# wenz116/lang2seg

Measured on AMD Instinct MI355X. Metric: train images/sec (cycle loss on), 600×1000 input, at 1/2/4/8 MI355X, higher is better.
Workload: dtype bf16; 1 GPU; train_cycle.sh step: ResNet-101 C4 + 7 spatial dynamic filters + att2in2 cycle loss, 600x1000 image, 20-token expression (V=3349), 12000->2000 proposals, 256 RoIs, per-GPU batch 1; variant=cycle, parallelism=dp1

## Files before the change

lang2seg_amd/csrc/conv_igemm.hip:

```cpp
#include "common.h"
#include "roi_sample.h"
#include "../../include/lang2seg_hip.h"
#include <stdlib.h>

namespace {

template <typename T> struct Mma;
template <> struct Mma<bf16_t> {
  static __device__ __forceinline__ f32x4 run(const uint4& a, const uint4& b, f32x4 c) {
    return __builtin_amdgcn_mfma_f32_16x16x32_bf16(__builtin_bit_cast(bf16x8, a), __builtin_bit_cast(bf16x8, b), c, 0, 0, 0);
  }
};
template <> struct Mma<float> {
  static __device__ __forceinline__ f32x4 run(const uint4& a, const uint4& b, f32x4 c) {
    c = __builtin_amdgcn_mfma_f32_16x16x4f32(__uint_as_float(a.x), __uint_as_float(b.x), c, 0, 0, 0);
    c = __builtin_amdgcn_mfma_f32_16x16x4f32(__uint_as_float(a.y), __uint_as_float(b.y), c, 0, 0, 0);
    c = __builtin_amdgcn_mfma_f32_16x16x4f32(__uint_as_float(a.z), __uint_as_float(b.z), c, 0, 0, 0);
    c = __builtin_amdgcn_mfma_f32_16x16x4f32(__uint_as_float(a.w), __uint_as_float(b.w), c, 0, 0, 0);
    return c;
  }
};

constexpr int ROWB = 128;
constexpr int LROW = ROWB + 16;
// ... 699 lines not shown
    __syncthreads();
    int t0 = 0;
    for (; t0 + 2 * D <= KT; t0 += D) {
#pragma unroll
      for (int s = 0; s < D; ++s) {
        const int t = t0 + s;
        const int nxt = (s + 1) % D;
        store_slice((t + 1) & 1, ra[nxt], rb[nxt]);
        issue(ra[nxt], rb[nxt]);
        __syncthreads();
      }
    }
#pragma unroll
    for (int s = 0; s < 2 * D; ++s) {
      const int t = t0 + s;
      if (t + 1 < KT) {
        const int nxt = (s + 1) % D;
        store_slice((t + 1) & 1, ra[nxt], rb[nxt]);
        if (t + 1 + D < KT) issue(ra[nxt], rb[nxt]);
        __syncthreads();
      }
    }
    return;
  }

  const int tid = (int)threadIdx.x, lane = tid & 63, wave = wave_all;
  const int wm = wave >> 1, wn = wave & 1;
  const int fr = lane & 15, fg = lane >> 4;
  const bool plain = !(p.flags & (L2S_CONV_DECONV2X2 | L2S_CONV_SCATTER)) && !(p.ldy & 7) && !(p.ldadd & 7) && !(p.ldref & 7) && !(p.Cout & 7) &&
                     !((uintptr_t)p.y & 15) && !((uintptr_t)p.add & 15) && !((uintptr_t)p.ref & 15) && !((uintptr_t)p.bias & 15) &&
                     (long)M * p.ldy * 2 < (1L << 31) && (!p.add || (long)M * p.ldadd * 2 < (1L << 31)) && (!p.ref || (long)M * p.ldref * 2 < (1L << 31));
  const bool staged = plain && gridDim.z == 1;
  constexpr int EIT = (BM * (BN / 8) + 255) / 256;
  u32x4v eav[EIT], erv[EIT];
  const bool pre = staged;
  if (pre && KT >= 8) igemm_epilogue_prefetch<BM, 256, BN>(p, m0, n0, M, tid, eav, erv);
  f32x4 ebv[BN / 32];
#pragma unroll
  for (int j = 0; j < BN / 32; ++j) {
    const int n = n0 + (wave_all & 1) * (BN / 2) + j * 16 + (lane >> 4) * 4;
    ebv[j] = (f32x4){0.f, 0.f, 0.f, 0.f};
    if (staged && p.bias && n < p.Cout) ebv[j] = *(const f32x4*)(p.bias + n);
  }
  const int swz = fr & (CPR - 1);
  const int offa = (wm * WM + fr) * RB, offb = BM * RB + (wn * WN + fr) * RB;
  f32x4 acc[TM][TN];
#pragma unroll
  for (int i = 0; i < TM; ++i)
#pragma unroll
    for (int j = 0; j < TN; ++j) acc[i][j] = (f32x4){0.f, 0.f, 0.f, 0.f};
  uint4 fa0[KG][TM], fb0[KG][TN], fa1[KG][TM], fb1[KG][TN];
  auto read_all = [&](int t, uint4 (&fa)[KG][TM], uint4 (&fb)[KG][TN]) {
    const char* base = smem + (t & 1) * BUF;
#pragma unroll
    for (int kg = 0; kg < KG; ++kg) {
      const int ch = ((kg * 4 + fg) ^ swz) << 4;
#pragma unroll
      for (int i = 0; i < TM; ++i) fa[kg][i] = *(const uint4*)(base + offa + i * 16 * RB + ch);
#pragma unroll
      for (int j = 0; j < TN; ++j) fb[kg][j] = *(const uint4*)(base + offb + j * 16 * RB + ch);
    }
  };
  auto mma_all = [&](const uint4 (&fa)[KG][TM], const uint4 (&fb)[KG][TN]) {
#pragma unroll
    for (int kg = 0; kg < KG; ++kg)
#pragma unroll
      for (int i = 0; i < TM; ++i)
#pragma unroll
        for (int j = 0; j < TN; ++j) acc[i][j] = Mma<T>::run(fb[kg][j], fa[kg][i], acc[i][j]);
  };
  __syncthreads();
  unsigned long long t_first = 0, t_loop = 0;
  if constexpr (STAMP) t_first = __builtin_amdgcn_s_memrealtime();
  read_all(0, fa0, fb0);
  if (pre && KT < 8) igemm_epilogue_prefetch<BM, 256, BN>(p, m0, n0, M, tid, eav, erv);
  int t = 1;
  for (; t + 2 <= KT; t += 2) {
    __syncthreads(); read_all(t, fa1, fb1); mma_all(fa0, fb0);
    __syncthreads(); read_all(t + 1, fa0, fb0); mma_all(fa1, fb1);
  }
  if (t < KT) { __syncthreads(); read_all(t, fa1, fb1); mma_all(fa0, fb0); mma_all(fa1, fb1); }
  else mma_all(fa0, fb0);
  if (gridDim.z > 1) { igemm_splitk_slab<TM, TN, WM, WN>(p, acc, m0, n0, wm, wn, fr, fg, M); return; }
  if constexpr (STAMP) {
    asm volatile("s_nop 0" : "+v"(acc[0][0]), "+v"(acc[TM - 1][TN - 1]));
    t_loop = __builtin_amdgcn_s_memrealtime();
  }
  if (staged) {
    igemm_epilogue_lds128<TM, TN, WM, WN, 2, 256, BN, 1>(p, acc, m0, n0, wm, wn, fr, fg, M, smem_all, eav, erv, ebv);
    if constexpr (STAMP) {
      asm volatile("s_waitcnt vmcnt(0)" ::: "memory");
      if (tid == 0 && p.ws) {
        unsigned long long* o = (unsigned long long*)p.ws + 4L * (blockIdx.x + (long)gridDim.x * blockIdx.z);
        o[0] = t_entry; o[1] = t_first; o[2] = t_loop; o[3] = __builtin_amdgcn_s_memrealtime();
      }
    }
    return;
  }
  igemm_epilogue<T, TM, TN, WM, WN, false>(p, acc, m0, n0, wm, wn, fr, fg, M);
}

template <typename T, int BM, int BN, int WGM, int WGN, int D, bool OUTF32, bool TAPIN>
__global__ __launch_bounds__(64 * WGM * WGN) void igemm_sp_kernel(const l2s_conv_desc p) {
  constexpr int VE = 16 / (int)sizeof(T);
  constexpr int BK = ROWB / (int)sizeof(T);
  constexpr int NTG = 64 * WGM * WGN, LR = NTG / 8;
  constexpr int WM = BM / WGM, WN = BN / WGN, TM = WM / 16, TN = WN / 16;
  constexpr int NA = (BM + LR - 1) / LR, NB = BN / LR;
  constexpr int BUF = (BM + BN) * ROWB;
  static_assert(D >= 2, "ring depth");
  extern __shared__ __attribute__((aligned(16))) char smem[];

  const int tid = threadIdx.x, lane = tid & 63, wave = tid >> 6;
  const int wm = wave / WGN, wn = wave % WGN;
  const int M = p.n_img * p.OH * p.OW;
  const int K = p.KH * p.KW * p.Cin;
  int mt, nt;
  {
    const int MT = (M + BM - 1) / BM, NT = (p.Cout + BN - 1) / BN, G = MT * NT;
    const int L = blockIdx.x, x = L & 7, slot = L >> 3, q = G >> 3, r = G & 7;
    const int t = x * q + min(x, r) + slot;
    if (p.xcd_mode == 0) { mt = t / NT; nt = t - mt * NT; } else { nt = t / MT; mt = t - nt * MT; }
  }
  const int m0 = mt * BM, n0 = nt * BN;
  const long xpix = (long)p.n_img * p.IH * p.IW;
  const auto rx = __builtin_amdgcn_make_buffer_rsrc((void*)p.x, 0, (int)(((xpix - 1) * p.ldx + p.Cin) * (long)sizeof(T)), 0x00020000);
  const auto rw = __builtin_amdgcn_make_buffer_rsrc((void*)p.w, 0, (int)((long)p.Cout * K * (long)sizeof(T)), 0x00020000);

  const int lrow = tid >> 3, cv = tid & 7;
  const int wchunk = ((cv ^ (lrow & 7)) << 4);
  int a_iy0[NA], a_ix0[NA], a_base[NA]; bool a_ok[NA];
  const int ohw = p.OH * p.OW;
#pragma unroll
  for (int j = 0; j < NA; ++j) {
    int m = m0 + lrow + LR * j;
    a_ok[j] = m < M && (lrow + LR * j) < BM;
    int mm = a_ok[j] ? m : 0;
    int n_img = mm / ohw, rem = mm - n_img * ohw;
    int oy = rem / p.OW, ox = rem - oy * p.OW;
    a_iy0[j] = oy * p.stride - p.pad;
    a_ix0[j] = ox * p.stride - p.pad;
    a_base[j] = n_img * p.IH * p.IW;
  }
  unsigned voffB[NB];
#pragma unroll
  for (int j = 0; j < NB; ++j) {
    const int n = n0 + lrow + LR * j;
    voffB[j] = n < p.Cout ? (unsigned)(((long)n * K + cv * VE) * (long)sizeof(T)) : OOR;
  }
  const int KT = K / BK;
  const int taps = p.KH * p.KW;
  int it = 0, c0 = 0, tap = 0;
  unsigned voffA[NA];
  int vbase[NA]; unsigned tmask[NA];
  auto set_tap = [&](int t) {
    const int ky = t / p.KW, kx = t - ky * p.KW;
#pragma unroll
    for (int j = 0; j < NA; ++j) {
      const int iy = a_iy0[j] + ky, ix = a_ix0[j] + kx;
      const bool v = a_ok[j] && iy >= 0 && iy < p.IH && ix >= 0 && ix < p.IW;
      voffA[j] = v ? (unsigned)(((long)(a_base[j] + iy * p.IW + ix) * p.ldx + cv * VE) * (long)sizeof(T)) : OOR;
    }
  };
  if (TAPIN) {
#pragma unroll
    for (int j = 0; j < NA; ++j) {
      vbase[j] = ((a_base[j] + a_iy0[j] * p.IW + a_ix0[j]) * p.ldx + cv * VE) * (int)sizeof(T);
      unsigned m = 0;
      for (int t = 0; t < taps; ++t) {
        const int ky = t / p.KW, kx = t - ky * p.KW;
        const int iy = a_iy0[j] + ky, ix = a_ix0[j] + kx;
        if (a_ok[j] && iy >= 0 && iy < p.IH && ix >= 0 && ix < p.IW) m |= 1u << t;
      }
      tmask[j] = m;
    }
  } else {
    set_tap(0);
  }
  auto issue = [&](uint4 (&a)[NA], uint4 (&b)[NB]) {
    int sa, sb;
    if (TAPIN) {
      const int ky = tap / p.KW, kx = tap - ky * p.KW;
      const int toff = (ky * p.IW + kx) * p.ldx * (int)sizeof(T);
      sa = c0 * (int)sizeof(T); sb = (tap * p.Cin + c0) * (int)sizeof(T);
#pragma unroll
      for (int j = 0; j < NA; ++j) voffA[j] = ((tmask[j] >> tap) & 1u) ? (unsigned)(vbase[j] + toff) : OOR;
    } else {
      sa = c0 * (int)sizeof(T); sb = it * (BK * (int)sizeof(T));
    }
#pragma unroll
    for (int j = 0; j < NA; ++j) a[j] = __builtin_bit_cast(uint4, __builtin_amdgcn_raw_buffer_load_b128(rx, voffA[j], sa, 0));
#pragma unroll
    for (int j = 0; j < NB; ++j) b[j] = __builtin_bit_cast(uint4, __builtin_amdgcn_raw_buffer_load_b128(rw, voffB[j], sb, 0));
    ++it;
    if (TAPIN) {
      if (++tap == taps) { tap = 0; c0 += BK; }
    } else {
      c0 += BK;
      if (c0 >= p.Cin && taps > 1) { c0 = 0; ++tap; if (tap < taps) set_tap(tap); }
    }
  };
  auto store_slice = [&](int buf, const uint4 (&ra)[NA], const uint4 (&rb)[NB]) {
    char* a = smem + buf * BUF + lrow * ROWB + wchunk;
    char* b = a + BM * ROWB;
#pragma unroll
    for (int j = 0; j < NA; ++j) if ((BM % LR) == 0 || j < NA - 1 || lrow < (BM % LR)) *(uint4*)(a + LR * j * ROWB) = ra[j];
#pragma unroll
    for (int j = 0; j < NB; ++j) *(uint4*)(b + LR * j * ROWB) = rb[j];
  };

  f32x4 acc[TM][TN];
#pragma unroll
  for (int i = 0; i < TM; ++i)
#pragma unroll
    for (int j = 0; j < TN; ++j) acc[i][j] = (f32x4){0.f, 0.f, 0.f, 0.f};

  const int fr = lane & 15, fg = lane >> 4;
  const int swz = fr & 7;
  const int offa = (wm * WM + fr) * ROWB, offb = BM * ROWB + (wn * WN + fr) * ROWB;
  const int ch0 = ((0 * 4 + fg) ^ swz) << 4, ch1 = ((1 * 4 + fg) ^ swz) << 4;
  auto read_frags = [&](int buf, int ch, uint4 (&fa)[TM], uint4 (&fb)[TN]) {
    const char* base = smem + buf * BUF;
#pragma unroll
    for (int i = 0; i < TM; ++i) fa[i] = *(const uint4*)(base + offa + i * 16 * ROWB + ch);
#pragma unroll
    for (int j = 0; j < TN; ++j) fb[j] = *(const uint4*)(base + offb + j * 16 * ROWB + ch);
  };
  auto mma = [&](const uint4 (&fa)[TM], const uint4 (&fb)[TN]) {
#pragma unroll
    for (int i = 0; i < TM; ++i)
#pragma unroll
      for (int j = 0; j < TN; ++j) acc[i][j] = Mma<T>::run(fb[j], fa[i], acc[i][j]);
  };

  uint4 ra[D][NA], rb[D][NB];
#pragma unroll
  for (int s = 0; s < D; ++s)
    if (s < KT) issue(ra[s], rb[s]);
  store_slice(0, ra[0], rb[0]);
  if (D < KT) issue(ra[0], rb[0]);
  if (1 < KT) {
    store_slice(1, ra[1], rb[1]);
    if (D + 1 < KT) issue(ra[1], rb[1]);
  }
  __syncthreads();
  uint4 fa0[TM], fb0[TN], fa1[TM], fb1[TN];
  read_frags(0, ch0, fa0, fb0);

  int t0 = 0, b0 = 0;
  for (; t0 + 2 * D + 2 <= KT; t0 += D) {
#pragma unroll
    for (int s = 0; s < D; ++s) {
      const int set = (s + 2) % D;
      const int bt = b0, bt1 = b0 == 2 ? 0 : b0 + 1, bt2 = bt1 == 2 ? 0 : bt1 + 1;
      if (s > 0 || t0 > 0) __syncthreads();
      read_frags(bt, ch1, fa1, fb1);
      store_slice(bt2, ra[set], rb[set]);
      issue(ra[set], rb[set]);
      mma(fa0, fb0);
      read_frags(bt1, ch0, fa0, fb0);
      mma(fa1, fb1);
      b0 = bt1;
    }
  }
#pragma unroll
  for (int s = 0; s < 2 * D + 2; ++s) {
    const int t = t0 + s;
    if (t < KT) {
      const int set = (s + 2) % D;
      const int bt = b0, bt1 = b0 == 2 ? 0 : b0 + 1, bt2 = bt1 == 2 ? 0 : bt1 + 1;
      if (t > 0) __syncthreads();
      read_frags(bt, ch1, fa1, fb1);
      if (t + 2 < KT) {
        store_slice(bt2, ra[set], rb[set]);
        if (t + 2 + D < KT) issue(ra[set], rb[set]);
      }
      mma(fa0, fb0);
      if (t + 1 < KT) read_frags(bt1, ch0, fa0, fb0);
      mma(fa1, fb1);
      b0 = bt1;
    }
  }
  if constexpr (sizeof(T) == 2 && !OUTF32 && BN == 128) {
    const bool plain = !(p.flags & (L2S_CONV_DECONV2X2 | L2S_CONV_SCATTER)) && !(p.ldy & 7) && !(p.ldadd & 7) && !(p.ldref & 7) && !(p.Cout & 7) &&
                       !((uintptr_t)p.y & 15) && !((uintptr_t)p.add & 15) && !((uintptr_t)p.ref & 15) && !((uintptr_t)p.bias & 15) &&
                       (long)M * p.ldy * 2 < (1L << 31) && (!p.add || (long)M * p.ldadd * 2 < (1L << 31)) && (!p.ref || (long)M * p.ldref * 2 < (1L << 31));
    if (plain) { igemm_epilogue_lds128<TM, TN, WM, WN, WGM, NTG, BN, 1>(p, acc, m0, n0, wm, wn, fr, fg, M, smem); return; }
  }
  igemm_epilogue<T, TM, TN, WM, WN, OUTF32>(p, acc, m0, n0, wm, wn, fr, fg, M);
}

typedef int i32x4s __attribute__((ext_vector_type(4)));
__device__ __forceinline__ void dma_b128(const i32x4s& rsrc, unsigned voff, unsigned soff, unsigned lds) {
  asm volatile("s_mov_b32 m0, %3\n\ts_nop 0\n\tbuffer_load_dwordx4 %0, %1, %2 offen lds" ::"v"(voff), "s"(rsrc), "s"(soff), "s"(lds) : "memory");
}
__device__ __forceinline__ void wg_barrier() { asm volatile("s_barrier" ::: "memory"); }
__device__ __forceinline__ void wait_lgkm0() { asm volatile("s_waitcnt lgkmcnt(0)" ::: "memory"); }

template <int BM, int BN, bool STAMP = false>
__global__ __launch_bounds__(512) void igemm_dma_kernel(const l2s_conv_desc p) {
  typedef bf16_t T;
  constexpr int WGM = 4, WGN = 2, WM = BM / WGM, WN = BN / WGN, TM = WM / 16, TN = WN / 16;
  constexpr int PA = BM / 64, PB = BN / 64, NP = PA + PB;
  constexpr int STG = (BM + BN) * ROWB;
  extern __shared__ __attribute__((aligned(16))) char smem[];
  const int tid = threadIdx.x, lane = tid & 63;
  const int wave = __builtin_amdgcn_readfirstlane(tid >> 6);
  const int grp = wave >> 2;
  const int wm = wave >> 1, wn = wave & 1;
  const int M = p.n_img * p.OH * p.OW;
  const int K = p.KH * p.KW * p.Cin;
  int mt, nt;
  {
    const int MT = (M + BM - 1) / BM, NT = (p.Cout + BN - 1) / BN, G = MT * NT;
    const int L = blockIdx.x, x = L & 7, slot = L >> 3, q = G >> 3, r = G & 7;
    const int t = x * q + min(x, r) + slot;
    if (p.xcd_mode == 0) { mt = t / NT; nt = t - mt * NT; } else { nt = t / MT; mt = t - nt * MT; }
  }
  const int m0 = mt * BM, n0 = nt * BN;
  const unsigned lds0 = (unsigned)(uintptr_t)(__attribute__((address_space(3))) char*)smem;
  const long xpix = (long)p.n_img * p.IH * p.IW;
  i32x4s rx, rw;
  rx.x = (int)(uintptr_t)p.x; rx.y = (int)((uintptr_t)p.x >> 32); rx.z = (int)(((xpix - 1) * p.ldx + p.Cin) * 2L); rx.w = 0x00020000;
  rw.x = (int)(uintptr_t)p.w; rw.y = (int)((uintptr_t)p.w >> 32); rw.z = (int)((long)p.Cout * K * 2L); rw.w = 0x00020000;

  const int prow = lane >> 3, sch = (lane & 7) ^ prow;
  const int ohw = p.OH * p.OW;
  int vbase[PA]; unsigned ntmask[PA];
#pragma unroll
  for (int j = 0; j < PA; ++j) {
    const int m = m0 + 8 * (wave + 8 * j) + prow;
    const bool ok = m < M;
    const int mm = ok ? m : 0;
    const int n_img = mm / ohw, rem = mm - n_img * ohw;
    const int oy = rem / p.OW, ox = rem - oy * p.OW;
    const int iy0 = oy * p.stride - p.pad, ix0 = ox * p.stride - p.pad;
    vbase[j] = (((n_img * p.IH + iy0) * p.IW + ix0) * p.ldx + sch * 8) * 2;
    unsigned mk = 0;
#pragma unroll
    for (int ky = 0; ky < 3; ++ky)
#pragma unroll
      for (int kx = 0; kx < 3; ++kx) {
        const int iy = iy0 + ky, ix = ix0 + kx;
        if (ky < p.KH && kx < p.KW && ok && iy >= 0 && iy < p.IH && ix >= 0 && ix < p.IW) mk |= 1u << (ky * p.KW + kx);
      }
    ntmask[j] = ~mk;
  }
  unsigned voffB[PB];
#pragma unroll
  for (int j = 0; j < PB; ++j) {
    const int n = n0 + 8 * (wave + 8 * j) + prow;
    voffB[j] = n < p.Cout ? (unsigned)(((long)n * K + sch * 8) * 2L) : OOR;
  }
  const int KT = K / 64;
  int c0 = 0, ky = 0, kx = 0, tapi = 0;
  unsigned vo[PA], soA = 0, soB = 0;
  int toff = 0;
  auto prep_s = [&]() {
    toff = (ky * p.IW + kx) * p.ldx * 2;
    soA = (unsigned)(c0 * 2); soB = (unsigned)((tapi * p.Cin + c0) * 2);
  };
#ifdef L2S_TOOLS
  const bool ko_a = (p.prio >> 8) & 1;
  auto prep_v = [&](int j) { vo[j] = ((((ntmask[j] >> tapi) & 1u) | (unsigned)(ko_a && tapi != 0)) << 31) | (unsigned)(vbase[j] + toff); asm volatile("" : "+v"(vo[j])); };
#else
  auto prep_v = [&](int j) { vo[j] = (((ntmask[j] >> tapi) & 1u) << 31) | (unsigned)(vbase[j] + toff); asm volatile("" : "+v"(vo[j])); };
#endif
  auto prep_adv = [&]() {
    const int nkx = kx + 1; const bool wx = nkx == p.KW; kx = wx ? 0 : nkx;
    const int nky = ky + (wx ? 1 : 0); const bool wy = nky == p.KH; ky = wy ? 0 : nky;
    tapi = wy ? 0 : tapi + 1; c0 += wy ? 64 : 0;
  };
  auto prep = [&]() {
    prep_s();
#pragma unroll
    for (int j = 0; j < PA; ++j) prep_v(j);
    prep_adv();
  };
  const unsigned ldsA = lds0 + (unsigned)(wave * 1024), ldsB = ldsA + (unsigned)(BM * ROWB);
  auto request = [&](int stage) {
    const unsigned sb = (unsigned)(stage * STG);
#pragma unroll
    for (int j = 0; j < PA; ++j) dma_b128(rx, vo[j], soA, ldsA + sb + (unsigned)(j * 8192));
#pragma unroll
    for (int j = 0; j < PB; ++j) dma_b128(rw, voffB[j], soB, ldsB + sb + (unsigned)(j * 8192));
  };

  f32x4 acc[TM][TN];
#pragma unroll
  for (int i = 0; i < TM; ++i)
#pragma unroll
    for (int j = 0; j < TN; ++j) acc[i][j] = (f32x4){0.f, 0.f, 0.f, 0.f};
  const int fr = lane & 15, fg = lane >> 4;
  const int swz = fr & 7;
  const int offa = (wm * WM + fr) * ROWB, offb = BM * ROWB + (wn * WN + fr) * ROWB;
  uint4 fa[2][TM], fb[2][TN];
  auto read_all = [&](int stage) {
    const char* base = smem + stage * STG;
#pragma unroll
    for (int kg = 0; kg < 2; ++kg) {
      const int ch = ((kg * 4 + fg) ^ swz) << 4;
#pragma unroll
      for (int i = 0; i < TM; ++i) fa[kg][i] = *(const uint4*)(base + offa + i * 16 * ROWB + ch);
#pragma unroll
      for (int j = 0; j < TN; ++j) fb[kg][j] = *(const uint4*)(base + offb + j * 16 * ROWB + ch);
    }
  };
  auto mma_all = [&]() {
    int q = 0;
#pragma unroll
    for (int kg = 0; kg < 2; ++kg)
#pragma unroll
      for (int i = 0; i < TM; ++i)
#pragma unroll
        for (int j = 0; j < TN; ++j) {
          acc[i][j] = Mma<T>::run(fb[kg][j], fa[kg][i], acc[i][j]);
          if (q == 2) { __builtin_amdgcn_sched_barrier(0); prep_s(); __builtin_amdgcn_sched_barrier(0); }
          if (q >= 6 && (q - 6) % 4 == 0 && (q - 6) / 4 < PA) { __builtin_amdgcn_sched_barrier(0); prep_v((q - 6) / 4); __builtin_amdgcn_sched_barrier(0); }
          if (q == 6 + 4 * PA) { __builtin_amdgcn_sched_barrier(0); prep_adv(); __builtin_amdgcn_sched_barrier(0); }
          ++q;
        }
  };

  prep(); request(0);
  if (1 < KT) { prep(); request(1); asm volatile("s_waitcnt vmcnt(%0)" ::"n"(NP) : "memory"); }
  else asm volatile("s_waitcnt vmcnt(0)" ::: "memory");
  if (2 < KT) prep();
  wg_barrier();
  if (grp == 1) wg_barrier();
  int st = 0;
  unsigned long long* stamps = (unsigned long long*)(smem + 3 * STG) + (grp * 24 * 8);
  const bool stamping = STAMP && blockIdx.x == 0 && (wave & 3) == 0 && lane == 0;
  const bool fine = STAMP && !(p.prio & 0x200);
  unsigned long long loop_c0 = 0, loop_r0 = 0;
  if constexpr (STAMP) { loop_c0 = __builtin_amdgcn_s_memtime(); loop_r0 = __builtin_amdgcn_s_memrealtime(); }
  auto stamp = [&](int t, int i) {
    if constexpr (STAMP) {
      if (fine && t < 24) {
        const unsigned long long c = __builtin_amdgcn_s_memtime(); if (stamping) stamps[t * 8 + i] = c;
        if (i == 0) { const unsigned long long r = __builtin_amdgcn_s_memrealtime(); if (stamping) ((unsigned long long*)(smem + 3 * STG))[2 * 24 * 8 + grp * 24 + t] = r; }
      }
    }
  };
  for (int t = 0; t < KT; ++t) {
    const int st2 = st == 0 ? 2 : st - 1;
    stamp(t, 0);
    read_all(st);
    stamp(t, 1);
    if (t + 2 < KT) request(st2);
    stamp(t, 2);
    wait_lgkm0();
    stamp(t, 3);
    if (grp == 1) {
      if (t + 2 < KT) asm volatile("s_waitcnt vmcnt(%0)" ::"n"(NP) : "memory");
      else asm volatile("s_waitcnt vmcnt(0)" ::: "memory");
    }
    wg_barrier();
    stamp(t, 4);
    __builtin_amdgcn_sched_barrier(0);
    mma_all();
    __builtin_amdgcn_sched_barrier(0);
    stamp(t, 5);
    if (grp == 0) {
      if (t + 2 < KT) asm volatile("s_waitcnt vmcnt(%0)" ::"n"(NP) : "memory");
      else asm volatile("s_waitcnt vmcnt(0)" ::: "memory");
    }
    stamp(t, 6);
    wg_barrier();
    stamp(t, 7);
    st = st == 2 ? 0 : st + 1;
  }
  if (grp == 0) wg_barrier();
  if constexpr (STAMP) {
    const unsigned long long loop_c1 = __builtin_amdgcn_s_memtime(), loop_r1 = __builtin_amdgcn_s_memrealtime();
    if (stamping) {
      unsigned long long* o = (unsigned long long*)(smem + 3 * STG) + 2 * 24 * 8 + 48 + grp * 2;
      o[0] = loop_c1 - loop_c0; o[1] = loop_r1 - loop_r0;
    }
    __syncthreads();
    if (blockIdx.x == 0 && tid < 2 * 24 * 8 + 2 * 24 + 4 && p.ws) ((unsigned long long*)p.ws)[tid] = ((unsigned long long*)(smem + 3 * STG))[tid];
    __syncthreads();
  }
  {
    const bool plain = !(p.flags & (L2S_CONV_DECONV2X2 | L2S_CONV_SCATTER)) && !(p.ldy & 7) && !(p.ldadd & 7) && !(p.ldref & 7) && !(p.Cout & 7) &&
                       !((uintptr_t)p.y & 15) && !((uintptr_t)p.add & 15) && !((uintptr_t)p.ref & 15) && !((uintptr_t)p.bias & 15) &&
                       (long)M * p.ldy * 2 < (1L << 31) && (!p.add || (long)M * p.ldadd * 2 < (1L << 31)) && (!p.ref || (long)M * p.ldref * 2 < (1L << 31));
    if (plain) { igemm_epilogue_lds128<TM, TN, WM, WN, WGM, 512, BN, 1>(p, acc, m0, n0, wm, wn, fr, fg, M, smem); return; }
  }
  igemm_epilogue<T, TM, TN, WM, WN, false>(p, acc, m0, n0, wm, wn, fr, fg, M);
}

constexpr int T196 = 196, R208 = 208;
template <int TMW>
__device__ __forceinline__ void igemm_dma196_body(const l2s_conv_desc& p, char* smem, int wave, int lane) {
  typedef bf16_t T;
  constexpr int BM = 256, BN = 128, TN = 4;
  constexpr int PA = BM / 64, PB = BN / 64, NP = PA + PB;
  constexpr int STG = (BM + BN) * ROWB;
  const int tid = threadIdx.x;
  const int grp = wave >> 2;
  const int wm = wave >> 1, wn = wave & 1;
  const int rbase = wm == 0 ? 0 : 16 + 48 * wm;
  const int M = p.n_img * p.OH * p.OW;
  const int K = p.KH * p.KW * p.Cin;
  int mt, nt;
  {
    const int MT = (M + T196 - 1) / T196, NT = (p.Cout + BN - 1) / BN, G = MT * NT;
    const int L = blockIdx.x, x = L & 7, slot = L >> 3, q = G >> 3, r = G & 7;
    const int t = x * q + min(x, r) + slot;
    if (p.xcd_mode == 0) { mt = t / NT; nt = t - mt * NT; } else { nt = t / MT; mt = t - nt * MT; }
  }
  const int m0 = mt * T196, n0 = nt * BN;
  const unsigned lds0 = (unsigned)(uintptr_t)(__attribute__((address_space(3))) char*)smem;
  const long xpix = (long)p.n_img * p.IH * p.IW;
  i32x4s rx, rw;
  rx.x = (int)(uintptr_t)p.x; rx.y = (int)((uintptr_t)p.x >> 32); rx.z = (int)(((xpix - 1) * p.ldx + p.Cin) * 2L); rx.w = 0x00020000;
  rw.x = (int)(uintptr_t)p.w; rw.y = (int)((uintptr_t)p.w >> 32); rw.z = (int)((long)p.Cout * K * 2L); rw.w = 0x00020000;
  const int prow = lane >> 3, sch = (lane & 7) ^ prow;
  const int ohw = p.OH * p.OW;
  int vbase[PA]; unsigned ntmask[PA];
#pragma unroll
  for (int j = 0; j < PA; ++j) {
    const int lr = 8 * (wave + 8 * j) + prow;
    const int m = m0 + lr;
    const bool ok = m < M && lr < R208;
    const int mm = ok ? m : 0;
    const int n_img = mm / ohw, rem = mm - n_img * ohw;
    const int oy = rem / p.OW, ox = rem - oy * p.OW;
    const int iy0 = oy * p.stride - p.pad, ix0 = ox * p.stride - p.pad;
    vbase[j] = (((n_img * p.IH + iy0) * p.IW + ix0) * p.ldx + sch * 8) * 2;
    unsigned mk = 0;
#pragma unroll
    for (int ky = 0; ky < 3; ++ky)
#pragma unroll
      for (int kx = 0; kx < 3; ++kx) {
        const int iy = iy0 + ky, ix = ix0 + kx;
        if (ky < p.KH && kx < p.KW && ok && iy >= 0 && iy < p.IH && ix >= 0 && ix < p.IW) mk |= 1u << (ky * p.KW + kx);
      }
    ntmask[j] = ~mk;
  }
  unsigned voffB[PB];
#pragma unroll
  for (int j = 0; j < PB; ++j) {
    const int n = n0 + 8 * (wave + 8 * j) + prow;
    voffB[j] = n < p.Cout ? (unsigned)(((long)n * K + sch * 8) * 2L) : OOR;
  }
  const int KT = K / 64;
  int c0 = 0, ky = 0, kx = 0, tapi = 0;
  unsigned vo[PA], soA = 0, soB = 0;
  int toff = 0;
  auto prep_s = [&]() {
    toff = (ky * p.IW + kx) * p.ldx * 2;
    soA = (unsigned)(c0 * 2); soB = (unsigned)((tapi * p.Cin + c0) * 2);
  };
  auto prep_v = [&](int j) { vo[j] = (((ntmask[j] >> tapi) & 1u) << 31) | (unsigned)(vbase[j] + toff); asm volatile("" : "+v"(vo[j])); };
  auto prep_adv = [&]() {
    const int nkx = kx + 1; const bool wx = nkx == p.KW; kx = wx ? 0 : nkx;
    const int nky = ky + (wx ? 1 : 0); const bool wy = nky == p.KH; ky = wy ? 0 : nky;
    tapi = wy ? 0 : tapi + 1; c0 += wy ? 64 : 0;
  };
  auto prep = [&]() {
    prep_s();
#pragma unroll
    for (int j = 0; j < PA; ++j) prep_v(j);
    prep_adv();
  };
  const unsigned ldsA = lds0 + (unsigned)(wave * 1024), ldsB = ldsA + (unsigned)(BM * ROWB);
  auto request = [&](int stage) {
    const unsigned sb = (unsigned)(stage * STG);
#pragma unroll
    for (int j = 0; j < PA; ++j) dma_b128(rx, vo[j], soA, ldsA + sb + (unsigned)(j * 8192));
#pragma unroll
    for (int j = 0; j < PB; ++j) dma_b128(rw, voffB[j], soB, ldsB + sb + (unsigned)(j * 8192));
  };
  f32x4 acc[TMW][TN];
#pragma unroll
  for (int i = 0; i < TMW; ++i)
#pragma unroll
    for (int j = 0; j < TN; ++j) acc[i][j] = (f32x4){0.f, 0.f, 0.f, 0.f};
  const int fr = lane & 15, fg = lane >> 4;
  const int swz = fr & 7;
  const int offa = (rbase + fr) * ROWB, offb = BM * ROWB + (wn * 64 + fr) * ROWB;
  uint4 fa[2][TMW], fb[2][TN];
  auto read_all = [&](int stage) {
    const char* base = smem + stage * STG;
#pragma unroll
    for (int kg = 0; kg < 2; ++kg) {
      const int ch = ((kg * 4 + fg) ^ swz) << 4;
#pragma unroll
      for (int i = 0; i < TMW; ++i) fa[kg][i] = *(const uint4*)(base + offa + i * 16 * ROWB + ch);
#pragma unroll
      for (int j = 0; j < TN; ++j) fb[kg][j] = *(const uint4*)(base + offb + j * 16 * ROWB + ch);
    }
  };
  auto mma_all = [&]() {
    int q = 0;
#pragma unroll
    for (int kg = 0; kg < 2; ++kg)
#pragma unroll
      for (int i = 0; i < TMW; ++i)
#pragma unroll
        for (int j = 0; j < TN; ++j) {
          acc[i][j] = Mma<T>::run(fb[kg][j], fa[kg][i], acc[i][j]);
          if (q == 2) { __builtin_amdgcn_sched_barrier(0); prep_s(); __builtin_amdgcn_sched_barrier(0); }
          if (q >= 5 && (q - 5) % 4 == 0 && (q - 5) / 4 < PA) { __builtin_amdgcn_sched_barrier(0); prep_v((q - 5) / 4); __builtin_amdgcn_sched_barrier(0); }
          if (q == 5 + 4 * PA) { __builtin_amdgcn_sched_barrier(0); prep_adv(); __builtin_amdgcn_sched_barrier(0); }
          ++q;
        }
  };
  prep(); request(0);
  if (1 < KT) { prep(); request(1); asm volatile("s_waitcnt vmcnt(%0)" ::"n"(NP) : "memory"); }
  else asm volatile("s_waitcnt vmcnt(0)" ::: "memory");
  if (2 < KT) prep();
  wg_barrier();
  if (grp == 1) wg_barrier();
  int st = 0;
  for (int t = 0; t < KT; ++t) {
    const int st2 = st == 0 ? 2 : st - 1;
    read_all(st);
    if (t + 2 < KT) request(st2);
    wait_lgkm0();
    if (grp == 1) {
      if (t + 2 < KT) asm volatile("s_waitcnt vmcnt(%0)" ::"n"(NP) : "memory");
      else asm volatile("s_waitcnt vmcnt(0)" ::: "memory");
    }
    wg_barrier();
    __builtin_amdgcn_sched_barrier(0);
    mma_all();
    __builtin_amdgcn_sched_barrier(0);
    if (grp == 0) {
      if (t + 2 < KT) asm volatile("s_waitcnt vmcnt(%0)" ::"n"(NP) : "memory");
      else asm volatile("s_waitcnt vmcnt(0)" ::: "memory");
    }
    wg_barrier();
    st = st == 2 ? 0 : st + 1;
  }
  if (grp == 0) wg_barrier();
  {
    constexpr int LDW = BN + 4, CPR = BN / 8, CH = R208 * CPR, NTH = 512, IT = (CH + NTH - 1) / NTH;
    constexpr unsigned NOPE = 0x80000000u;
    float* stg = (float*)smem;
    const auto ry = __builtin_amdgcn_make_buffer_rsrc((void*)p.y, 0, 0x7FFFFFFF, 0x00020000);
    const auto radd = __builtin_amdgcn_make_buffer_rsrc((void*)(p.add ? p.add : p.y), 0, 0x7FFFFFFF, 0x00020000);
    const auto rref = __builtin_amdgcn_make_buffer_rsrc((void*)(p.ref ? p.ref : p.y), 0, 0x7FFFFFFF, 0x00020000);
    f32x4 bv[TN];
#pragma unroll
    for (int j = 0; j < TN; ++j) {
      const int n = n0 + wn * 64 + j * 16 + fg * 4;
      bv[j] = (f32x4){0.f, 0.f, 0.f, 0.f};
      if (p.bias && n < p.Cout) bv[j] = *(const f32x4*)(p.bias + n);
    }
    __syncthreads();
#pragma unroll
    for (int i = 0; i < TMW; ++i)
#pragma unroll
      for (int j = 0; j < TN; ++j) {
        f32x4 v = acc[i][j];
        v[0] += bv[j][0]; v[1] += bv[j][1]; v[2] += bv[j][2]; v[3] += bv[j][3];
        *(f32x4*)(stg + (rbase + i * 16 + fr) * LDW + wn * 64 + j * 16 + fg * 4) = v;
      }
    __syncthreads();
    u32x4v av[IT], rv[IT];
    unsigned off[IT];
#pragma unroll
    for (int k = 0; k < IT; ++k) {
      const int c = tid + NTH * k, row = c / CPR, col = (c % CPR) * 8;
      const int m = m0 + row, n = n0 + col;
      const bool ok = c < CH && row < T196 && m < M && n < p.Cout;
      off[k] = ok ? (unsigned)m : NOPE;
      if (p.add) av[k] = __builtin_amdgcn_raw_buffer_load_b128(radd, ok ? (unsigned)((m * p.ldadd + n) * 2) : NOPE, 0, 0);
      if (p.ref) rv[k] = __builtin_amdgcn_raw_buffer_load_b128(rref, ok ? (unsigned)((m * p.ldref + n) * 2) : NOPE, 0, 0);
    }
#pragma unroll
    for (int k = 0; k < IT; ++k) {
      const int c = min(tid + NTH * k, CH - 1), row = c / CPR, col = (c % CPR) * 8;
      const f32x4 lo = *(const f32x4*)(stg + row * LDW + col), hi = *(const f32x4*)(stg + row * LDW + col + 4);
      float v[8] = {lo[0], lo[1], lo[2], lo[3], hi[0], hi[1], hi[2], hi[3]};
      if (p.add) {
        const unsigned w[4] = {av[k].x, av[k].y, av[k].z, av[k].w};
#pragma unroll
        for (int e = 0; e < 4; ++e) { v[2 * e] += __uint_as_float(w[e] << 16); v[2 * e + 1] += __uint_as_float(w[e] & 0xFFFF0000u); }
      }
      if (p.flags & L2S_CONV_RELU) {
#pragma unroll
        for (int e = 0; e < 8; ++e) v[e] = fmaxf(v[e], 0.f);
      }
      if (p.ref) {
        const unsigned w[4] = {rv[k].x, rv[k].y, rv[k].z, rv[k].w};
#pragma unroll
        for (int e = 0; e < 4; ++e) {
          if (!(__uint_as_float(w[e] << 16) > 0.f)) v[2 * e] = 0.f;
          if (!(__uint_as_float(w[e] & 0xFFFF0000u) > 0.f)) v[2 * e + 1] = 0.f;
        }
      }
      u32x4v pk;
      pk.x = (uint32_t)f2bf(v[0]) | ((uint32_t)f2bf(v[1]) << 16); pk.y = (uint32_t)f2bf(v[2]) | ((uint32_t)f2bf(v[3]) << 16);
      pk.z = (uint32_t)f2bf(v[4]) | ((uint32_t)f2bf(v[5]) << 16); pk.w = (uint32_t)f2bf(v[6]) | ((uint32_t)f2bf(v[7]) << 16);
      const int n = n0 + col;
      __builtin_amdgcn_raw_buffer_store_b128(pk, ry, off[k] != NOPE ? (unsigned)((off[k] * p.ldy + n) * 2) : NOPE, 0, 0);
    }
  }
}
__global__ __launch_bounds__(512) void igemm_dma196_kernel(const l2s_conv_desc p) {
  extern __shared__ __attribute__((aligned(16))) char smem[];
  const int lane = threadIdx.x & 63;
  const int wave = __builtin_amdgcn_readfirstlane(threadIdx.x >> 6);
  if ((wave >> 1) == 0) igemm_dma196_body<4>(p, smem, wave, lane);
  else igemm_dma196_body<3>(p, smem, wave, lane);
}

template <int TM, int TN, int WM, int WN>
__device__ __forceinline__ void igemm_epilogue_wave_prefetch(const l2s_conv_desc& p, int m0, int n0, int wm, int wn, int lane, int M, f32x4 (&bv)[TN], u32x2 (&ov)[TM][TN]) {
  constexpr unsigned NOPE = 0x80000000u;
  const int fr = lane & 15, fg = lane >> 4;
  const void* op = p.add ? p.add : p.ref;
  const int ldo = p.add ? p.ldadd : p.ldref;
  const auto rop = __builtin_amdgcn_make_buffer_rsrc((void*)(op ? op : p.y), 0, 0x7FFFFFFF, 0x00020000);
  const auto rbias = __builtin_amdgcn_make_buffer_rsrc((void*)(p.bias ? (const void*)p.bias : (const void*)p.y), 0, 0x7FFFFFFF, 0x00020000);
#pragma unroll
  for (int j = 0; j < TN; ++j) {
    const int n = n0 + wn * WN + j * 16 + fg * 4;
    bv[j] = __builtin_bit_cast(f32x4, __builtin_amdgcn_raw_buffer_load_b128(rbias, (p.bias && n < p.Cout) ? (unsigned)(n * 4) : NOPE, 0, 0));
  }
#pragma unroll
  for (int i = 0; i < TM; ++i) {
    const int m = m0 + wm * WM + i * 16 + fr;
#pragma unroll
    for (int j = 0; j < TN; ++j) {
      const int n = n0 + wn * WN + j * 16 + fg * 4;
      ov[i][j] = __builtin_amdgcn_raw_buffer_load_b64(rop, (op && m < M && n < p.Cout) ? (unsigned)(((long)m * ldo + n) * 2) : NOPE, 0, 0);
    }
  }
}
template <int TM, int TN, int WM, int WN>
__device__ __forceinline__ void igemm_epilogue_wave(const l2s_conv_desc& p, f32x4 (&acc)[TM][TN], int m0, int n0, int wm, int wn, int lane, int M, char* wlds,
                                                    const f32x4 (&bv)[TN], const u32x2 (&ov)[TM][TN]) {
  static_assert(TN == 4 && WN == 64, "64-channel sub-tiles");
  constexpr unsigned NOPE = 0x80000000u;
  const int fr = lane & 15, fg = lane >> 4;
  const auto ry = __builtin_amdgcn_make_buffer_rsrc((void*)p.y, 0, 0x7FFFFFFF, 0x00020000);
  const int wsw = (fr >> 1) & 7;
  const int rrow = lane >> 3, rch = lane & 7;
#pragma unroll
  for (int i = 0; i < TM; ++i) {
#pragma unroll
    for (int j = 0; j < TN; ++j) {
      float v[4] = {acc[i][j][0] + bv[j][0], acc[i][j][1] + bv[j][1], acc[i][j][2] + bv[j][2], acc[i][j][3] + bv[j][3]};
      const float o[4] = {__uint_as_float(ov[i][j].x << 16), __uint_as_float(ov[i][j].x & 0xFFFF0000u), __uint_as_float(ov[i][j].y << 16), __uint_as_float(ov[i][j].y & 0xFFFF0000u)};
      if (p.add) { v[0] += o[0]; v[1] += o[1]; v[2] += o[2]; v[3] += o[3]; }
      if (p.flags & L2S_CONV_RELU) { v[0] = fmaxf(v[0], 0.f); v[1] = fmaxf(v[1], 0.f); v[2] = fmaxf(v[2], 0.f); v[3] = fmaxf(v[3], 0.f); }
      if (p.ref) {
#pragma unroll
        for (int e = 0; e < 4; ++e) if (!(o[e] > 0.f)) v[e] = 0.f;
      }
      u32x2 pk;
      pk.x = (uint32_t)f2bf(v[0]) | ((uint32_t)f2bf(v[1]) << 16);
      pk.y = (uint32_t)f2bf(v[2]) | ((uint32_t)f2bf(v[3]) << 16);
      *(u32x2*)(wlds + fr * 128 + (((2 * j + (fg >> 1)) ^ wsw) << 4) + ((fg & 1) << 3)) = pk;
    }
#pragma unroll
    for (int h = 0; h < 2; ++h) {
      const int row = rrow + 8 * h;
      const u32x4v q = *(const u32x4v*)(wlds + row * 128 + ((rch ^ ((row >> 1) & 7)) << 4));
      const int m = m0 + wm * WM + i * 16 + row, n = n0 + wn * WN + rch * 8;
      const unsigned o = (m < M && n < p.Cout) ? (unsigned)(((long)m * p.ldy + n) * 2) : NOPE;
      __builtin_amdgcn_raw_buffer_store_b128(q, ry, o, 0, 0);
    }
  }
}

template <int TM, int TN, bool BOTH>
__device__ __forceinline__ void igemm_epilogue_wave128(const l2s_conv_desc& p, f32x4 (&acc)[TM][TN], int m0, int n0, int wm, int wn, int lane, int M, char* wlds) {
  static_assert(TN == 8, "128-channel sub-tiles");
  constexpr unsigned NOPE = 0x80000000u;
  constexpr int WM = TM * 16, WN = TN * 16;
  const int fr = lane & 15, fg = lane >> 4;
  const void* op = p.add ? p.add : p.ref;
  const int ldo = p.add ? p.ldadd : p.ldref;
  const auto rop = __builtin_amdgcn_make_buffer_rsrc((void*)(op ? op : p.y), 0, 0x7FFFFFFF, 0x00020000);
// ... 1045 lines not shown
```

Before: 223.4 img/s.

## Interleave LDS fragment reads and DMA loads with MFMAs in the DMA igemm loop

```diff
diff --git a/lang2seg_amd/csrc/conv_igemm.hip b/lang2seg_amd/csrc/conv_igemm.hip
--- a/lang2seg_amd/csrc/conv_igemm.hip
+++ b/lang2seg_amd/csrc/conv_igemm.hip
@@ -1025,11 +1025,12 @@
   typedef bf16_t T;
   constexpr int WGM = 4, WGN = 2, WM = BM / WGM, WN = BN / WGN, TM = WM / 16, TN = WN / 16;
   constexpr int PA = BM / 64, PB = BN / 64, NP = PA + PB;
+  constexpr int NF = TM + TN;
+  static_assert(NP == 6 && NF == 8 && TM * TN == 16, "the phase schedule is written for the 256 x 128 tile");
   constexpr int STG = (BM + BN) * ROWB;
   extern __shared__ __attribute__((aligned(16))) char smem[];
   const int tid = threadIdx.x, lane = tid & 63;
   const int wave = __builtin_amdgcn_readfirstlane(tid >> 6);
-  const int grp = wave >> 2;
   const int wm = wave >> 1, wn = wave & 1;
   const int M = p.n_img * p.OH * p.OW;
   const int K = p.KH * p.KW * p.Cin;
@@ -1101,12 +1102,10 @@
     prep_adv();
   };
   const unsigned ldsA = lds0 + (unsigned)(wave * 1024), ldsB = ldsA + (unsigned)(BM * ROWB);
-  auto request = [&](int stage) {
+  auto piece = [&](int stage, int q) __attribute__((always_inline)) {
     const unsigned sb = (unsigned)(stage * STG);
-#pragma unroll
-    for (int j = 0; j < PA; ++j) dma_b128(rx, vo[j], soA, ldsA + sb + (unsigned)(j * 8192));
-#pragma unroll
-    for (int j = 0; j < PB; ++j) dma_b128(rw, voffB[j], soB, ldsB + sb + (unsigned)(j * 8192));
+    if (q < PA) dma_b128(rx, vo[q], soA, ldsA + sb + (unsigned)(q * 8192));
+    else dma_b128(rw, voffB[q - PA], soB, ldsB + sb + (unsigned)((q - PA) * 8192));
   };
 
   f32x4 acc[TM][TN];
@@ -1117,87 +1116,92 @@
   const int fr = lane & 15, fg = lane >> 4;
   const int swz = fr & 7;
   const int offa = (wm * WM + fr) * ROWB, offb = BM * ROWB + (wn * WN + fr) * ROWB;
+  const int chk[2] = {((0 * 4 + fg) ^ swz) << 4, ((1 * 4 + fg) ^ swz) << 4};
   uint4 fa[2][TM], fb[2][TN];
-  auto read_all = [&](int stage) {
+  auto read_frag = [&](int stage, int kg, int f) __attribute__((always_inline)) {
     const char* base = smem + stage * STG;
-#pragma unroll
-    for (int kg = 0; kg < 2; ++kg) {
-      const int ch = ((kg * 4 + fg) ^ swz) << 4;
-#pragma unroll
-      for (int i = 0; i < TM; ++i) fa[kg][i] = *(const uint4*)(base + offa + i * 16 * ROWB + ch);
-#pragma unroll
-      for (int j = 0; j < TN; ++j) fb[kg][j] = *(const uint4*)(base + offb + j * 16 * ROWB + ch);
-    }
-  };
-  auto mma_all = [&]() {
-    int q = 0;
-#pragma unroll
-    for (int kg = 0; kg < 2; ++kg)
-#pragma unroll
-      for (int i = 0; i < TM; ++i)
-#pragma unroll
-        for (int j = 0; j < TN; ++j) {
-          acc[i][j] = Mma<T>::run(fb[kg][j], fa[kg][i], acc[i][j]);
-          if (q == 2) { __builtin_amdgcn_sched_barrier(0); prep_s(); __builtin_amdgcn_sched_barrier(0); }
-          if (q >= 6 && (q - 6) % 4 == 0 && (q - 6) / 4 < PA) { __builtin_amdgcn_sched_barrier(0); prep_v((q - 6) / 4); __builtin_amdgcn_sched_barrier(0); }
-          if (q == 6 + 4 * PA) { __builtin_amdgcn_sched_barrier(0); prep_adv(); __builtin_amdgcn_sched_barrier(0); }
-          ++q;
-        }
-  };
-
-  prep(); request(0);
-  if (1 < KT) { prep(); request(1); asm volatile("s_waitcnt vmcnt(%0)" ::"n"(NP) : "memory"); }
-  else asm volatile("s_waitcnt vmcnt(0)" ::: "memory");
-  if (2 < KT) prep();
-  wg_barrier();
-  if (grp == 1) wg_barrier();
-  int st = 0;
-  unsigned long long* stamps = (unsigned long long*)(smem + 3 * STG) + (grp * 24 * 8);
-  const bool stamping = STAMP && blockIdx.x == 0 && (wave & 3) == 0 && lane == 0;
+    if (f < TM) fa[kg][f] = *(const uint4*)(base + offa + f * 16 * ROWB + chk[kg]);
+    else fb[kg][f - TM] = *(const uint4*)(base + offb + (f - TM) * 16 * ROWB + chk[kg]);
+  };
+  auto phase = [&](int kg, bool rd, int rs, bool dn, int ds, int q0, bool pp) __attribute__((always_inline)) {
+#pragma unroll
+    for (int q = 0; q < 16; ++q) {
+      const int i = q / TN, j = q % TN;
+      acc[i][j] = Mma<T>::run(fb[kg][j], fa[kg][i], acc[i][j]);
+      __builtin_amdgcn_sched_barrier(0);
+      if (q < NF) { if (rd) read_frag(rs, kg ^ 1, q); }
+      else if (q < NF + 3) { if (dn) piece(ds, q0 + q - NF); }
+      else if (pp) {
+        if (q == NF + 3) prep_s();
+        if (q > NF + 3) prep_v(q - NF - 4);
+        if (q == 15) prep_adv();
+      }
+      __builtin_amdgcn_sched_barrier(0);
+    }
+  };
+  auto wait_vm = [&](bool more) {
+    if (more) asm volatile("s_waitcnt vmcnt(%0)" ::"n"(NP) : "memory");
+    else asm volatile("s_waitcnt vmcnt(0)" ::: "memory");
+  };
+
+  const int sw = wave >> 2;
+  unsigned long long* stamps = (unsigned long long*)(smem + 3 * STG) + (sw * 24 * 8);
+  const bool stamping = STAMP && blockIdx.x == 0 && (wave & 3) == 0;
   const bool fine = STAMP && !(p.prio & 0x200);
-  unsigned long long loop_c0 = 0, loop_r0 = 0;
-  if constexpr (STAMP) { loop_c0 = __builtin_amdgcn_s_memtime(); loop_r0 = __builtin_amdgcn_s_memrealtime(); }
-  auto stamp = [&](int t, int i) {
+  auto stamp = [&](int t, int i) __attribute__((always_inline)) {
     if constexpr (STAMP) {
       if (fine && t < 24) {
         const unsigned long long c = __builtin_amdgcn_s_memtime(); if (stamping) stamps[t * 8 + i] = c;
-        if (i == 0) { const unsigned long long r = __builtin_amdgcn_s_memrealtime(); if (stamping) ((unsigned long long*)(smem + 3 * STG))[2 * 24 * 8 + grp * 24 + t] = r; }
-      }
-    }
-  };
-  for (int t = 0; t < KT; ++t) {
-    const int st2 = st == 0 ? 2 : st - 1;
+        if (i == 0) { const unsigned long long r = __builtin_amdgcn_s_memrealtime(); if (stamping) ((unsigned long long*)(smem + 3 * STG))[2 * 24 * 8 + sw * 24 + t] = r; }
+      }
+    }
+  };
+
+  prep();
+#pragma unroll
+  for (int q = 0; q < NP; ++q) piece(0, q);
+  prep();
+#pragma unroll
+  for (int q = 0; q < NP; ++q) piece(1, q);
+  prep();
+#pragma unroll
+  for (int q = 0; q < 3; ++q) piece(2, q);
+  asm volatile("s_waitcnt vmcnt(%0)" ::"n"(NP + 3) : "memory");
+  wg_barrier();
+#pragma unroll
+  for (int f = 0; f < NF; ++f) read_frag(0, 0, f);
+  unsigned long long loop_c0 = 0, loop_r0 = 0;
+  if constexpr (STAMP) { loop_c0 = __builtin_amdgcn_s_memtime(); loop_r0 = __builtin_amdgcn_s_memrealtime(); }
+
+  auto slice = [&](int t, int st, bool n1, bool n2, bool n3) __attribute__((always_inline)) {
+    const int st1 = st == 2 ? 0 : st + 1, st2 = st1 == 2 ? 0 : st1 + 1;
     stamp(t, 0);
-    read_all(st);
+    phase(0, true, st, n2, st2, 3, n3);
     stamp(t, 1);
-    if (t + 2 < KT) request(st2);
-    stamp(t, 2);
     wait_lgkm0();
+    if (n1) {
+      wait_vm(n2);
+      stamp(t, 2);
+      wg_barrier();
+    }
     stamp(t, 3);
-    if (grp == 1) {
-      if (t + 2 < KT) asm volatile("s_waitcnt vmcnt(%0)" ::"n"(NP) : "memory");
-      else asm volatile("s_waitcnt vmcnt(0)" ::: "memory");
-    }
-    wg_barrier();
+    phase(1, n1, st1, n3, st, 0, false);
     stamp(t, 4);
-    __builtin_amdgcn_sched_barrier(0);
-    mma_all();
-    __builtin_amdgcn_sched_barrier(0);
-    stamp(t, 5);
-    if (grp == 0) {
-      if (t + 2 < KT) asm volatile("s_waitcnt vmcnt(%0)" ::"n"(NP) : "memory");
-      else asm volatile("s_waitcnt vmcnt(0)" ::: "memory");
-    }
-    stamp(t, 6);
-    wg_barrier();
-    stamp(t, 7);
+  };
+  int t = 0, st = 0;
+  for (; t + 3 < KT; ++t) {
+    slice(t, st, true, true, true);
     st = st == 2 ? 0 : st + 1;
   }
-  if (grp == 0) wg_barrier();
+  slice(t, st, true, true, false);
+  st = st == 2 ? 0 : st + 1;
+  slice(t + 1, st, true, false, false);
+  st = st == 2 ? 0 : st + 1;
+  slice(t + 2, st, false, false, false);
   if constexpr (STAMP) {
     const unsigned long long loop_c1 = __builtin_amdgcn_s_memtime(), loop_r1 = __builtin_amdgcn_s_memrealtime();
     if (stamping) {
-      unsigned long long* o = (unsigned long long*)(smem + 3 * STG) + 2 * 24 * 8 + 48 + grp * 2;
+      unsigned long long* o = (unsigned long long*)(smem + 3 * STG) + 2 * 24 * 8 + 48 + sw * 2;
       o[0] = loop_c1 - loop_c0; o[1] = loop_r1 - loop_r0;
     }
     __syncthreads();
```

Result: no change. 224.8 img/s (median of 6 runs) (+0.6%).
